# roclark/torchsr

Hardware: AMD Instinct MI355X
Metric: 96x96 HR crops/sec (SRGAN GAN train step) (higher is better)
Workload: dtype f32; 1 GPU; SRGAN full GAN step (Generator + Discriminator + VGG19 perceptual loss), 96x96 HR crops, batch 16 per GPU, fp32; per_gpu_batch=16, global_batch=16, crop=96, parallelism=dp1, hip_graph=True, vgg19_weights=seeded-random, plan_cus=256

## Files before the change

include/srx.h:

```cpp
#ifndef SRX_H
#define SRX_H

#include <stddef.h>
#include <stdint.h>

#ifdef __cplusplus
extern "C" {
#endif

#define SRX_VERSION 100

enum {
  SRX_OK = 0,
  SRX_E_BADARG = 1,
  SRX_E_UNSUPPORTED = 2,
  SRX_E_HIP = 3,
  SRX_E_WORKSPACE = 4
};

enum { SRX_ACT_NONE = 0, SRX_ACT_RELU = 1, SRX_ACT_LRELU = 2, SRX_ACT_PRELU = 3 };

int srx_version(void);
int srx_last_error(char* buf, size_t n);
int srx_build_info(char* buf, size_t n);
// ... 228 lines not shown
int srx_linear_bwd_data(const float* dy, const float* w, float* dx, int B, int K, int J, float* ws,
                        size_t ws_floats, void* stream);
int srx_linear_bwd_weight(const float* x, const float* dy, float* dw, int accumulate, int B, int K, int J,
                          void* stream);

int srx_mse_fwd(const float* a, const float* b, float* loss, int64_t n, float* ws, void* stream);
int srx_l1_fwd(const float* a, const float* b, float* loss, int64_t n, float* ws, void* stream);
int srx_mse_bwd(const float* a, const float* b, const float* gscale, float* da, float* db, int64_t n, void* stream);
int srx_l1_bwd(const float* a, const float* b, const float* gscale, float* da, float* db, int64_t n, void* stream);
int srx_l1_fwd_count(const float* a, const float* b, float* loss, int64_t n, int64_t count, float* ws, void* stream);
int srx_l1_bwd_count(const float* a, const float* b, const float* gscale, float* da, float* db, int64_t n, int64_t count,
                     void* stream);
int srx_bce_fwd(const float* p, float target, float* loss, int64_t n, float* ws, void* stream);
int srx_bce_bwd(const float* p, float target, const float* gscale, float* dp, int64_t n, void* stream);
int srx_bce_logits_fwd(const float* x, const float* shift, float target, float* loss, int64_t n, float* ws, void* stream);
int srx_bce_logits_bwd(const float* x, const float* shift, float target, const float* gscale, float* dx, int64_t n, void* stream);
int srx_mean_fwd(const float* x, float* out, int64_t n, float* ws, void* stream);
int srx_mean_bwd(const float* x, const float* gscale, float* dx, int64_t n, void* stream);

enum { SRX_HEAD_SRGAN_D = 0, SRX_HEAD_SRGAN_G = 1, SRX_HEAD_ESRGAN_D = 2, SRX_HEAD_ESRGAN_G = 3 };
typedef struct {
  int32_t mode, B, J, n_first;
  float slope, adv_weight;
} srx_gan_head_t;
int srx_gan_head_fwd(const srx_gan_head_t* h, const float* hidden, const float* w2, const float* b2, const float* shift,
                     const float* addend, float* zp, float* out, float* loss, void* stream);
int srx_gan_head_bwd(const srx_gan_head_t* h, const float* hidden, const float* w2, const float* zp, const float* out,
                     const float* shift, const float* g, float* dpre, float* dw2, float* db2, float* db1, int accumulate,
                     void* stream);

int srx_adam_step(float* p, const float* g, float* m, float* v, int64_t n, const float* lr, float beta1,
                  float beta2, float eps, float grad_scale, int64_t* step, void* stream);

#ifdef __cplusplus
}
#endif
#endif
```

torchsr_amd/_lib.py:

```python
import ctypes as C
import os
import subprocess
import sys

_HERE = os.path.dirname(os.path.abspath(__file__))
CSRC = os.path.join(_HERE, 'csrc')
LIB_PATH = os.environ.get('SRX_LIB') or os.path.join(CSRC, 'libsrx_hip.so')
SOURCES = ['api.cpp', 'gconv.hip', 'wgrad.hip', 'convpack.hip', 'c64.hip', 'thin9.hip', 'rdb.hip', 'thin.hip', 'rowtile.hip', 'augment.hip', 'norm.hip', 'eltwise.hip', 'linear.hip', 'loss.hip', 'head.hip', 'wino.hip', 'optim.hip']
HEADERS = ['srx_common.h', 'conv_host.h', os.path.join('..', '..', 'include', 'srx.h')]

ACT_NONE, ACT_RELU, ACT_LRELU, ACT_PRELU = 0, 1, 2, 3


class Conv2dDesc(C.Structure):
    _fields_ = [
        ('N', C.c_int32), ('H', C.c_int32), ('W', C.c_int32),
        ('Cin', C.c_int32), ('Cin_s', C.c_int32), ('Cout', C.c_int32), ('Cout_s', C.c_int32),
        ('KH', C.c_int32), ('KW', C.c_int32), ('stride', C.c_int32), ('pad', C.c_int32),
        ('shuffle', C.c_int32), ('act', C.c_int32), ('slope', C.c_float), ('up', C.c_int32),
        ('precision', C.c_int32),
    ]


class DgradEpilogue(C.Structure):
# ... 210 lines not shown
    'srx_mse_bwd': (_I, [_P, _P, _P, _P, _P, _L, _P]),
    'srx_l1_bwd': (_I, [_P, _P, _P, _P, _P, _L, _P]),
    'srx_l1_fwd_count': (_I, [_P, _P, _P, _L, _L, _P, _P]),
    'srx_l1_bwd_count': (_I, [_P, _P, _P, _P, _P, _L, _L, _P]),
    'srx_bce_fwd': (_I, [_P, _F, _P, _L, _P, _P]),
    'srx_bce_bwd': (_I, [_P, _F, _P, _P, _L, _P]),
    'srx_bce_logits_fwd': (_I, [_P, _P, _F, _P, _L, _P, _P]),
    'srx_bce_logits_bwd': (_I, [_P, _P, _F, _P, _P, _L, _P]),
    'srx_wino_applicable': (_I, [_D]),
    'srx_wino_packed_floats': (_Z, [_D]),
    'srx_wino_ws_floats': (_Z, [_D, _I]),
    'srx_wino_plan': (_I, [_D, _I, C.POINTER(C.c_int)]),
    'srx_wino_pack': (_I, [_D, _P, _P, _I, _P]),
    'srx_wino_fwd': (_I, [_D, _P, _P, _P, _P, _P, _Z, _P]),
    'srx_wino_bwd_data': (_I, [_D, _P, _P, _P, _P, _P, _Z, _P]),
    'srx_conv3x3_bf16s_applicable': (_I, [_D]),
    'srx_conv3x3_bf16s_packed_bytes': (_Z, [_D]),
    'srx_conv3x3_bf16s_pack': (_I, [_D, _P, _P, _P, _P]),
    'srx_conv3x3_bf16s_ws_floats': (_Z, [_D, _I]),
    'srx_conv3x3_bf16s_fwd': (_I, [_D, _P, _P, _P, _I, _P, _I, _P, _Z, _P]),
    'srx_conv3x3_bf16s_bwd_data': (_I, [_D, _P, _P, _P, _P, _I, _P, _Z, _P]),
    'srx_conv2d_fwd_first3_to_bf16': (_I, [_D, _P, _P, _P, _P, _P]),
    'srx_maxpool2x2_fwd_to_bf16': (_I, [_P, _P, _I, _I, _I, _I, _P]),
    'srx_maxpool2x2_relu_bwd_bf16': (_I, [_P, _P, _P, _I, _I, _I, _I, _P]),
    'srx_act_bwd_from_out_to_bf16': (_I, [_P, _P, _P, C.c_int64, _I, C.c_float, _P]),
    'srx_wino_infer_applicable': (_I, [_D]),
    'srx_wino_fwd_act': (_I, [_D, _P, _P, _P, _P, _P, _P, _Z, _P]),
    'srx_wino_force_plan': (_I, [_I, _I, _I]),
    'srx_wino_stat_rows': (_I, [_D]),
    'srx_wino_fwd_stats': (_I, [_D, _P, _P, _P, _P, _P, _P, _Z, _P]),
    'srx_gan_head_fwd': (_I, [C.POINTER(GanHead), _P, _P, _P, _P, _P, _P, _P, _P, _P]),
    'srx_gan_head_bwd': (_I, [C.POINTER(GanHead), _P, _P, _P, _P, _P, _P, _P, _P, _P, _P, _I, _P]),
    'srx_adam_step': (_I, [_P, _P, _P, _P, _L, _P, _F, _F, _F, _F, _P, _P]),
}
_UNCHECKED = {'srx_wino_applicable', 'srx_wino_infer_applicable', 'srx_conv3x3_bf16s_applicable', 'srx_wino_stat_rows', 'srx_conv2d_bwd_data_bn_rows', 'srx_conv2d_fwd_bn_in_ok', 'srx_conv2d_bwd_data_bn_in_ok', 'srx_pack_table_bytes', 'srx_version', 'srx_last_error', 'srx_device_cus', 'srx_plan_cus', 'srx_prof_stop', 'srx_conv2d_stat_rows', 'srx_bn_stat_rows', 'srx_bn_rows_per_block'}

EXPORTS = tuple(_SIGS.keys())

_lib = None


def load_handle(path: str) -> C.CDLL:
    import torch
    if torch.cuda.is_available():
        torch.cuda.init()
    return C.CDLL(path)


def _ensure_fresh():
    want = source_digest()
    if built_digest(LIB_PATH) == want:
        return
    import fcntl
    with open(os.path.join(CSRC, '.build.lock'), 'w') as lock:
        fcntl.flock(lock, fcntl.LOCK_EX)
        if built_digest(LIB_PATH) == want:
            return
        have = built_digest(LIB_PATH)
        print(f'torchsr_amd: {LIB_PATH} was built from other sources ({have and have[:12]} != {want[:12]}); rebuilding',
              file=sys.stderr)
        try:
            build()
        except (OSError, subprocess.CalledProcessError) as exc:
            raise RuntimeError(f'{LIB_PATH} is stale (built from sources {have and have[:12]}, the tree has {want[:12]}) and '
                               f'could not be rebuilt: {exc}.  Run `python -c "import __graft_entry__ as g; g.build()"`.') from exc


def lib() -> C.CDLL:
# ... 35 lines not shown
```

torchsr_amd/csrc/convpack.hip:

```cpp
#include "conv_host.h"

namespace {

__global__ void pack_fwd_kernel(const float* __restrict__ w, float* __restrict__ p, int Cout, int Cin, int KH, int KW,
                                int Ck, int K, int Kp, int Cnp, int shuffle_cps) {
  const int64_t idx = (int64_t)blockIdx.x * blockDim.x + threadIdx.x;
  if (idx >= (int64_t)Cnp * Kp) return;
  const int np = (int)(idx / Kp), k = (int)(idx - (int64_t)np * Kp);
  float v = 0.f;
  if (np < Cout && k < K) {
    const int tap = k / Ck, ci = k - tap * Ck;
    if (ci < Cin) {
      int co = np;
      if (shuffle_cps) { const int ij = np / shuffle_cps, cc = np - ij * shuffle_cps; co = cc * 4 + ij; }
      const int kh = tap / KW, kw = tap - kh * KW;
      v = w[(((size_t)co * Cin + ci) * KH + kh) * KW + kw];
    }
  }
  p[idx] = v;
}

__global__ void pack_bwd_kernel(const float* __restrict__ w, float* __restrict__ p, int Cout, int Cin, int KH, int KW,
                                int stride, int pad, int ph, int pw, int dminh, int dminw, int ntw, int Ck, int K,
                                int Kp, int Cnp, int shuffle_cps) {
// ... 196 lines not shown
      r.rows = Cnp; r.K = cls[c].K; r.Kp = cls[c].Kp; r.Ck = bwd_ck(d);
      r.ph = cls[c].ph; r.pw = cls[c].pw; r.dminh = cls[c].dminh; r.dminw = cls[c].dminw;
      r.ntw = cls[c].ntw > 0 ? cls[c].ntw : 1;
      r.n_elems = (long long)Cnp * (r.Ck + cls[c].Kp - cls[c].K);
      emit(r);
    }
  }
  *nrec_out = nrec;
  *max_elems_out = maxn;
  return SRX_OK;
}

extern "C" int srx_pack_table_add_wino(void* host_table, int* nrec, long long* max_elems, const srx_conv2d_t* d, const float* w,
                                       float* upk, int transpose) {
  SRX_REQUIRE(host_table && nrec && max_elems && d && w && upk && *nrec >= 0, "pack_table_add_wino: bad argument");
  SRX_REQUIRE(srx_wino_applicable(d) || srx_wino_packed_floats(d) > 0, "pack_table_add_wino: not a Winograd layer");
  PackRec r{};
  SRX_REQUIRE(!(transpose && d->shuffle), "pack_table_add_wino: a PixelShuffle layer has no Winograd data gradient");
  r.dst = upk; r.w = w; r.kind = transpose ? 5 : (d->shuffle ? 6 : 4);
  r.Cout = d->Cout; r.Cin = d->Cin; r.KH = 3; r.KW = 3; r.stride = 1; r.pad = 1;
  r.n_elems = (long long)d->Cout * d->Cin;
  static_cast<PackRec*>(host_table)[(*nrec)++] = r;
  if (r.n_elems > *max_elems) *max_elems = r.n_elems;
  return SRX_OK;
}

extern "C" int srx_pack_table_run(const void* dev_table, int nrec, long long max_elems, void* stream) {
  SRX_REQUIRE(dev_table && nrec > 0 && nrec <= 65535 && max_elems > 0, "pack_table_run: bad argument");
  hipLaunchKernelGGL(pack_table_kernel, dim3((unsigned)srx_cdiv(max_elems, 256), (unsigned)nrec), dim3(256), 0,
                     srx_stream(stream), static_cast<const PackRec*>(dev_table));
  SRX_CHECK_LAUNCH("pack_table_kernel");
  return SRX_OK;
}
```

torchsr_amd/csrc/optim.hip:

```cpp
#include "srx_common.h"

namespace {

__global__ void adam_tick_kernel(int64_t* step) { *step += 1; }

__global__ __launch_bounds__(256) void adam_kernel(float* __restrict__ p, const float* __restrict__ g,
                                                   float* __restrict__ m, float* __restrict__ v, int64_t n,
                                                   const float* __restrict__ lr_ptr, float beta1, float beta2,
                                                   float eps, float gscale, const int64_t* __restrict__ step_ptr) {
  const double t = (double)(*step_ptr);
  const float bc1 = (float)(1.0 - pow((double)beta1, t));
  const float bc2 = (float)(1.0 - pow((double)beta2, t));
  const float step_size = lr_ptr[0] / bc1;
  const float bc2_sqrt = sqrtf(bc2);
  const int64_t n4 = n / 4;
  for (int64_t i = (int64_t)blockIdx.x * blockDim.x + threadIdx.x; i < n4; i += (int64_t)gridDim.x * blockDim.x) {
    f32x4 pv = *reinterpret_cast<const f32x4*>(p + i * 4);
    f32x4 gv = *reinterpret_cast<const f32x4*>(g + i * 4);
    f32x4 mv = *reinterpret_cast<const f32x4*>(m + i * 4);
    f32x4 vv = *reinterpret_cast<const f32x4*>(v + i * 4);
#pragma unroll
    for (int e = 0; e < 4; ++e) {
      const float gg = gv[e] * gscale;
      mv[e] = beta1 * mv[e] + (1.f - beta1) * gg;
      vv[e] = beta2 * vv[e] + (1.f - beta2) * gg * gg;
      const float denom = sqrtf(vv[e]) / bc2_sqrt + eps;
      pv[e] -= step_size * (mv[e] / denom);
    }
    *reinterpret_cast<f32x4*>(p + i * 4) = pv;
    *reinterpret_cast<f32x4*>(m + i * 4) = mv;
    *reinterpret_cast<f32x4*>(v + i * 4) = vv;
  }
  if (blockIdx.x == 0 && threadIdx.x < (n & 3)) {
    const int64_t i = n4 * 4 + threadIdx.x;
    const float gg = g[i] * gscale;
    const float mm = beta1 * m[i] + (1.f - beta1) * gg;
    const float vv = beta2 * v[i] + (1.f - beta2) * gg * gg;
    m[i] = mm;
    v[i] = vv;
    p[i] -= step_size * (mm / (sqrtf(vv) / bc2_sqrt + eps));
  }
}

}

extern "C" int srx_adam_step(float* p, const float* g, float* m, float* v, int64_t n, const float* lr, float beta1,
                             float beta2, float eps, float grad_scale, int64_t* step, void* stream) {
  SRX_REQUIRE(p && g && m && v && lr && step && n > 0, "adam_step: bad argument");
  SRX_REQUIRE(((uintptr_t)p % 16 == 0) && ((uintptr_t)g % 16 == 0) && ((uintptr_t)m % 16 == 0) &&
                  ((uintptr_t)v % 16 == 0),
              "adam_step: buffers must be 16-byte aligned");
  hipStream_t st = srx_stream(stream);
  hipLaunchKernelGGL(adam_tick_kernel, dim3(1), dim3(1), 0, st, step);
  SRX_CHECK_LAUNCH("adam_tick_kernel");
  int64_t blocks = srx_cdiv(n / 4, 256);
  if (blocks > 4096) blocks = 4096;
  if (blocks < 1) blocks = 1;
  hipLaunchKernelGGL(adam_kernel, dim3((unsigned)blocks), dim3(256), 0, st, p, g, m, v, n, lr, beta1, beta2, eps,
                     grad_scale, step);
  SRX_CHECK_LAUNCH("adam_kernel");
  return SRX_OK;
}
```

torchsr_amd/csrc/srx_common.h:

```cpp
#pragma once
#include <hip/hip_runtime.h>
#include <hip/hip_ext.h>
#include <stdint.h>
#include <stddef.h>
#include "../../include/srx.h"

typedef float f32x4 __attribute__((ext_vector_type(4)));
typedef float f32x16 __attribute__((ext_vector_type(16)));

void srx_set_error(const char* fmt, ...);

#define SRX_FAIL(code, ...)      \
  do {                           \
    srx_set_error(__VA_ARGS__);  \
    return (code);               \
  } while (0)

#define SRX_REQUIRE(cond, ...) \
  do {                         \
    if (!(cond)) SRX_FAIL(SRX_E_BADARG, __VA_ARGS__); \
  } while (0)

#define SRX_CHECK_LAUNCH(name)                                                        \
  do {                                                                                \
// ... 41 lines not shown
                        const float* res;
                        float* z_out; };
struct srx_rt36_bnb_t { const float* y; const float* mean; const float* invstd; const float* gamma; const float* beta;
                        const float* prelu; const float* sums; float inv_m; float* dy_out; };
int srx_rt36_run(const srx_conv2d_t* d, const float* in, const float* wpk, const float* bias, const float* residual,
                 float* out, float* part, int act, float slope, hipStream_t st, const srx_rt36_bn_t* bn = nullptr,
                 const srx_rt36_bnl_t* bnl = nullptr, const srx_rt36_bnb_t* bnb = nullptr);

static inline hipStream_t srx_stream(void* s) { return (hipStream_t)s; }
static inline int64_t srx_cdiv(int64_t a, int64_t b) { return (a + b - 1) / b; }
static inline int64_t srx_roundup(int64_t a, int64_t b) { return srx_cdiv(a, b) * b; }

__device__ __forceinline__ void srx_divmod(int m, int d, float inv_d, int& q, int& r) {
  q = __float2int_rz(__int2float_rn(m) * inv_d);
  r = m - q * d;
  if (r < 0) { q -= 1; r += d; }
  if (r >= d) { q += 1; r -= d; }
}

__device__ __forceinline__ __amdgpu_buffer_rsrc_t srx_rsrc(const void* p, unsigned bytes) {
  return __builtin_amdgcn_make_buffer_rsrc(const_cast<void*>(p), (short)0, (int)bytes, 0x00020000);
}
__device__ __forceinline__ f32x4 srx_bload(__amdgpu_buffer_rsrc_t r, unsigned voff, unsigned soff) {
  return __builtin_bit_cast(f32x4, __builtin_amdgcn_raw_buffer_load_b128(r, (int)voff, (int)soff, 0));
}
__device__ __forceinline__ int srx_uniform(int v) { return __builtin_amdgcn_readfirstlane(v); }

__device__ __forceinline__ float srx_wave_sum(float v) {
#pragma unroll
  for (int o = 32; o > 0; o >>= 1) v += __shfl_xor(v, o, 64);
  return v;
}

__device__ __forceinline__ void srx_wino_pack_one(const float* __restrict__ w, float* __restrict__ upk, int Cout, int Cin,
                                                  int transpose, int64_t idx) {
  const int R = transpose == 1 ? Cin : Cout, K = transpose == 1 ? Cout : Cin;
  const int r = (int)(idx / K), k = (int)(idx - (int64_t)r * K);
  const int rsrc = transpose == 2 ? (r % (Cout / 4)) * 4 + r / (Cout / 4) : r;
  float g[3][3];
#pragma unroll
  for (int i = 0; i < 3; ++i)
#pragma unroll
    for (int j = 0; j < 3; ++j)
      g[i][j] = transpose == 1 ? w[(((size_t)k * Cin + r) * 3 + (2 - i)) * 3 + (2 - j)] : w[(((size_t)rsrc * Cin + k) * 3 + i) * 3 + j];
  float t[4][3];
#pragma unroll
  for (int j = 0; j < 3; ++j) {
    t[0][j] = g[0][j];
    t[1][j] = 0.5f * (g[0][j] + g[1][j] + g[2][j]);
    t[2][j] = 0.5f * (g[0][j] - g[1][j] + g[2][j]);
    t[3][j] = g[2][j];
  }
  const int nch = K / 32, rt = R / 32;
  const int jg = r >> 5, mrow = r & 31, kc = k / 32, kk = k % 32, quad = kk >> 2, e = kk & 3, s = quad >> 1, hh = quad & 1;
#pragma unroll
  for (int i = 0; i < 4; ++i) {
    const float u[4] = {t[i][0], 0.5f * (t[i][0] + t[i][1] + t[i][2]), 0.5f * (t[i][0] - t[i][1] + t[i][2]), t[i][2]};
#pragma unroll
    for (int j = 0; j < 4; ++j) {
      const int xi = 4 * i + j;
      upk[(((((size_t)xi * rt + jg) * nch + kc) * 4 + s) * 64 + hh * 32 + mrow) * 4 + e] = u[j];
    }
  }
}
```

torchsr_amd/functional.py:

```python
import contextlib
from typing import Optional, Tuple

import torch
from torch import Tensor
from torch.autograd import Function

from . import _dev, _lib
from ._lib import (ACT_LRELU, ACT_NONE, ACT_PRELU, ACT_RELU, HEAD_ESRGAN_D, HEAD_ESRGAN_G, HEAD_SRGAN_D, HEAD_SRGAN_G,
                   Conv2dDesc, call)

import ctypes as C


direct_grads = [False]


def _sink(param: Optional[Tensor]) -> Optional[Tensor]:
    if not direct_grads[0] or param is None or not param.requires_grad:
        return None
    g = param.grad
    if g is None or not g.is_cuda or g.dtype != torch.float32 or not g.is_contiguous():
        return None
    return g

# ... 319 lines not shown

    def pack_bf16s(self, weight: Tensor, d: Conv2dDesc, need_bwd: bool) -> None:
        key = self.pack_key(weight)
        have = self.__dict__.get('bf16s_fwd')
        if key == self.__dict__.get('_bf16s_key') and have is not None and (self.__dict__.get('bf16s_bwd') is not None or not need_bwd):
            return
        dref = C.byref(d)
        n = _lib.lib().srx_conv3x3_bf16s_packed_bytes(dref) // 2
        if have is None or have.device != weight.device:
            self.bf16s_fwd = torch.empty(n, dtype=torch.bfloat16, device=weight.device)
            self.bf16s_bwd = None
        if need_bwd and self.__dict__.get('bf16s_bwd') is None:
            self.bf16s_bwd = torch.empty(n, dtype=torch.bfloat16, device=weight.device)
        w = _chk(weight.detach(), 'conv2d.weight')
        call('srx_conv3x3_bf16s_pack', dref, _p(w), _p(self.bf16s_fwd), _p(self.bf16s_bwd), _stream())
        self._bf16s_key = key


def wino_forward_only_ok(st: ConvState, d: Conv2dDesc) -> bool:
    return (not _dev.NO_WINO and st.shuffle == 2 and st.act == ACT_NONE and st.precision == 0
            and _lib.lib().srx_wino_infer_applicable(C.byref(d)) == 1)


def wino_layer_ok(st: ConvState, d: Conv2dDesc) -> bool:
    return (not _dev.NO_WINO and st.act in (ACT_NONE, ACT_RELU) and _lib.lib().srx_wino_applicable(C.byref(d)) == 1)


def wino_forward_runs(st: ConvState, d: Conv2dDesc, want_stats: bool) -> bool:
    return wino_layer_ok(st, d) and (not want_stats or st.act == ACT_NONE)


class PackTable:

    def __init__(self, convs):
        self.convs = list(convs)
        self.table = None
        self.nrec, self.maxn = 0, 0
        self.fused_sig = None
        self.generation = 0

    def _build(self) -> bool:
        every = [(c._st, c.weight) for c in self.convs if c.weight.requires_grad and not c._st.fused_only]
        direct = [(st, wt) for st, wt in every if st.wpk_fwd is not None and getattr(st, 'last_desc', None) is not None]
        wino = [(st, wt) for st, wt in every if st.__dict__.get('wino_fwd') is not None]
        seen = {id(st) for st, _ in direct} | {id(st) for st, _ in wino}
        if not direct or any(id(st) not in seen for st, _ in every):
            return False
        items = direct
        n = len(items)
        descs = (Conv2dDesc * n)(*[st.last_desc for st, _ in items])
        arr = lambda ptrs: (C.c_void_p * n)(*ptrs)
        w, f, b = (arr([wt.data_ptr() for _, wt in items]), arr([st.wpk_fwd.data_ptr() for st, _ in items]),
                   arr([st.wpk_bwd.data_ptr() for st, _ in items]))
        nbytes = _lib.lib().srx_pack_table_bytes(n + len(wino))
        host = torch.empty(nbytes, dtype=torch.uint8)
        nrec, maxn = C.c_int(0), C.c_longlong(0)
        call('srx_pack_table_build', descs, n, w, f, b, host.data_ptr(), C.byref(nrec), C.byref(maxn))
        self.wino_items = wino
        for st, wt in self.wino_items:
            dref = C.byref(st._wino_desc)
            call('srx_pack_table_add_wino', host.data_ptr(), C.byref(nrec), C.byref(maxn), dref, wt.data_ptr(), st.wino_fwd.data_ptr(), 0)
            if st.wino_bwd is not None:
                call('srx_pack_table_add_wino', host.data_ptr(), C.byref(nrec), C.byref(maxn), dref, wt.data_ptr(), st.wino_bwd.data_ptr(), 1)
        self.table = host.to(items[0][1].device)
        self.items, self.nrec, self.maxn = items, nrec.value, maxn.value
        self.fused_sig = self._fused_signature()
        self.generation += 1
        return True

    def _fused_signature(self):
        return tuple((bool(c._st.fused_only), c._st.wpk_fwd is not None, c._st.__dict__.get('wino_fwd') is not None,
                      c._st.__dict__.get('wino_bwd') is not None) for c in self.convs)

    def run(self) -> bool:
        if self.table is not None and self.fused_sig != self._fused_signature():
            if torch.cuda.is_current_stream_capturing():
                raise RuntimeError('PackTable: the set of fused-only convs changed inside a hipGraph capture; run one eager step '
                                   'after switching precision / SRX_NO_RDB_FUSED')
            self.table = None
        if self.table is None and (torch.cuda.is_current_stream_capturing() or not self._build()):
            return False
        call('srx_pack_table_run', self.table.data_ptr(), self.nrec, self.maxn, _stream())
        for st, wt in self.items:
            st._key = st.pack_key(wt)
        for st, wt in self.wino_items:
            st._wino_key = st.pack_key(wt)
        return True


_pack_epoch = [0]


def bump_pack_epoch() -> None:
    _pack_epoch[0] += 1


class ActFold:
    __slots__ = ('act', 'slope', 'masked', 'consumers')

    def __init__(self, act: int, slope: float):
        self.act, self.slope, self.masked, self.consumers = act, float(slope), False, 0


class _Conv2d(Function):
    @staticmethod
    def forward(ctx, x: Tensor, weight: Tensor, bias: Optional[Tensor], st: ConvState, want_stats: bool,
                master: Tensor, in_act: Optional[ActFold] = None, act_bwd_folded: Optional[ActFold] = None):
        ctx.set_materialize_grads(False)
        if in_act is not None:
            if not isinstance(in_act, ActFold):
                raise TypeError('conv2d: in_act must be the ActFold token the producer was called with')
            in_act.consumers += 1
            if in_act.consumers > 1:
                raise RuntimeError('conv2d: an ActFold token has one consumer; this producer output feeds a second conv')
        if act_bwd_folded is not None and not isinstance(act_bwd_folded, ActFold):
            raise TypeError('conv2d: act_bwd_folded must be an ActFold token shared with the consumer')
        ctx.in_act, ctx.act_bwd_folded = in_act, act_bwd_folded
        x = _chk(x, 'conv2d.input')
        n, h, w, cs = x.shape
# ... 1645 lines not shown
```

torchsr_amd/optim.py:

```python
from typing import Iterable, List

import torch
from torch import nn, Tensor

from . import functional as F
from ._lib import call


class FlatParams:

    ALIGN = 4

    def __init__(self, module: nn.Module):
        params = [p for p in module.parameters() if p.requires_grad]
        if not params:
            raise RuntimeError('FlatParams: module has no trainable parameters')
        dev, dt = params[0].device, params[0].dtype
        if dt != torch.float32:
            raise RuntimeError('FlatParams: fp32 parameters expected')
        offs, total = [], 0
        for p in params:
            offs.append(total)
            total += (p.numel() + self.ALIGN - 1) // self.ALIGN * self.ALIGN
        self.data = torch.zeros(total, dtype=dt, device=dev)
# ... 10 lines not shown
            for p, o in zip(params, offs):
                n = p.numel()
                self.data[o:o + n].copy_(p.detach().reshape(-1))
                p.data = self.data[o:o + n].view(p.shape)
                p.grad = self.grad[o:o + n].view(p.shape)

    def offsets_by_name(self, module: nn.Module) -> dict:
        where = {id(p): o for p, o in zip(self.params, self.offsets)}
        return {n: where[id(p)] for n, p in module.named_parameters() if id(p) in where}

    def zero_grad(self) -> None:
        self.grad.zero_()
        off = 0
        for p in self.params:
            n = p.numel()
            if p.grad is None or p.grad.data_ptr() != self.grad.data_ptr() + off * 4:
                p.grad = self.grad[off:off + n].view(p.shape)
            off += (n + self.ALIGN - 1) // self.ALIGN * self.ALIGN


class FlatAdam:

    def __init__(self, flat: FlatParams, lr: float = 1e-4, betas=(0.9, 0.999), eps: float = 1e-8):
        self.flat = flat
        self.betas, self.eps = betas, eps
        dev = flat.data.device
        self.exp_avg = torch.zeros_like(flat.data)
        self.exp_avg_sq = torch.zeros_like(flat.data)
        self.step_count = torch.zeros((), dtype=torch.int64, device=dev)
        self.lr_dev = torch.tensor(float(lr), dtype=torch.float32, device=dev)
        self._lr = float(lr)
        self.grad_scale = 1.0
        self.pack_table = None
        self.param_groups = [{'lr': float(lr), 'initial_lr': float(lr)}]

    @property
    def lr(self) -> float:
        return self._lr

    def set_lr(self, lr: float) -> None:
        self._lr = float(lr)
        self.param_groups[0]['lr'] = float(lr)
        self.lr_dev.fill_(float(lr))

    def zero_grad(self) -> None:
        self.flat.zero_grad()

    @torch.no_grad()
    def step(self) -> None:
        f = self.flat
        call('srx_adam_step', f.data.data_ptr(), f.grad.data_ptr(), self.exp_avg.data_ptr(),
             self.exp_avg_sq.data_ptr(), f.numel, self.lr_dev.data_ptr(), self.betas[0], self.betas[1], self.eps,
             self.grad_scale, self.step_count.data_ptr(), torch.cuda.current_stream().cuda_stream)
        self.flat.pack_epoch[0] += 1
        if self.pack_table is not None:
            self.pack_table.run()

    def state_dict(self):
        return {'exp_avg': self.exp_avg, 'exp_avg_sq': self.exp_avg_sq, 'step': self.step_count, 'lr': self._lr}

    def load_state_dict(self, sd) -> None:
        self.exp_avg.copy_(sd['exp_avg'])
        self.exp_avg_sq.copy_(sd['exp_avg_sq'])
        self.step_count.copy_(sd['step'])
        self.set_lr(sd['lr'])


class StepLR:

    def __init__(self, optimizer: FlatAdam, step_size: int, gamma: float = 0.1):
        self.optimizer, self.step_size, self.gamma = optimizer, max(1, int(step_size)), gamma
        self.base_lr = optimizer.lr
        self.last_epoch = 0

    def step(self) -> None:
        self.last_epoch += 1
        self.optimizer.set_lr(self.base_lr * self.gamma ** (self.last_epoch // self.step_size))

    def get_last_lr(self):
        return [self.optimizer.lr]

    def state_dict(self):
        return {'last_epoch': self.last_epoch, 'base_lr': self.base_lr}

    def load_state_dict(self, sd) -> None:
        self.last_epoch, self.base_lr = sd['last_epoch'], sd['base_lr']
# ... 2 lines not shown
```

torchsr_amd/srgan/trainer.py:

```python
import os
import time
from argparse import Namespace
from math import log10
from typing import Callable, Dict, Optional

import torch
import torch.distributed as dist
from torch import Tensor

from .. import _dev
from .. import functional as F
from ..ddp import BackwardCuts, GradBuckets, broadcast_module
from ..layers import no_weight_grad, set_conv_precision
from ..optim import FlatAdam, FlatParams, StepLR
from .discriminator import Discriminator
from .generator import Generator
from .loss import VGGLoss

try:
    import wandb
except ImportError:
    wandb = None


# ... 126 lines not shown
        precision = 'bf16' if (self.amp and phase in self.amp_phases) else 'fp32'
        for module in (self.generator, self.discriminator, self.vgg_loss):
            set_conv_precision(module, precision)

    def _initialize_models(self) -> None:
        self.generator = self.generator_cls().to(self.device)
        self.discriminator = self.discriminator_cls().to(self.device)
        if self.distributed:
            broadcast_module(self.generator)
            broadcast_module(self.discriminator)
        self.gen_flat = FlatParams(self.generator)
        self.disc_flat = FlatParams(self.discriminator)
        force = self.force_collectives
        kw = {'force': force, 'reserve_cus': self.comm_reserved_cus, 'window_hook': self.comm_window_hook}
        self.gen_sync = GradBuckets(self.gen_flat, (self.gen_tail_bucket,), self.generator, **kw) if self.distributed else None
        self.disc_sync = GradBuckets(self.disc_flat, (self.disc_head_bucket,), self.discriminator, **kw) \
            if self.distributed else None

    def _initialize_loss(self) -> None:
        self.mse_loss = F.mse_loss
        self.pixel_loss = F.mse_loss
        self.bce_loss = F.bce_loss
        self.vgg_loss = VGGLoss(weights=self.vgg_weights).to(self.device)

    def _initialize_optimizers(self) -> None:
        self.psnr_optimizer = FlatAdam(self.gen_flat, lr=0.0001, betas=(0.9, 0.999))
        self.disc_optimizer = FlatAdam(self.disc_flat, lr=0.0001, betas=(0.9, 0.999))
        self.gen_optimizer = FlatAdam(self.gen_flat, lr=0.0001, betas=(0.9, 0.999))
        if self.distributed:
            for opt in (self.psnr_optimizer, self.gen_optimizer):
                opt.grad_scale = self.gen_sync.scale
            self.disc_optimizer.grad_scale = self.disc_sync.scale
        from ..layers import Conv2d
        gen_table = F.PackTable(m for m in self.generator.modules() if isinstance(m, Conv2d))
        disc_table = F.PackTable(m for m in self.discriminator.modules() if isinstance(m, Conv2d))
        self.psnr_optimizer.pack_table = self.gen_optimizer.pack_table = gen_table
        self.disc_optimizer.pack_table = disc_table
        self.disc_scheduler = StepLR(self.disc_optimizer, step_size=self.epochs // 8, gamma=0.6)
        self.gen_scheduler = StepLR(self.gen_optimizer, step_size=self.epochs // 8, gamma=0.6)

    def _create_test_image(self) -> None:
        path = 'media/waterfalls-low-res.png'
        if os.path.exists(path):
            import numpy as np
            from PIL import Image
            a = np.asarray(Image.open(path).convert('RGB'), dtype='float32') / 255.0
            image = torch.from_numpy(a).permute(2, 0, 1).contiguous()
        else:
            yy, xx = torch.meshgrid(torch.linspace(0, 1, 320), torch.linspace(0, 1, 480), indexing='ij')
            image = torch.stack([xx, yy, 0.5 + 0.5 * torch.sin(12 * xx * yy)])
        self.test_image = image.unsqueeze(0).to(self.device)

    def _log(self, statement: str) -> None:
        if self.main_process:
            print(statement)

    def _log_wandb(self, contents: dict, step: int = None) -> None:
        if wandb and self.main_process and getattr(wandb, 'run', None) is not None:
            wandb.log({k: (v.item() if torch.is_tensor(v) else v) for k, v in contents.items()}, step=step)

    def _cleanup(self) -> None:
        if wandb and getattr(wandb, 'run', None) is not None:
            wandb.finish()

    def _model_state(self, epoch: int, phase: str) -> dict:
        cpu = lambda sd: {k: (v.detach().clone().cpu() if torch.is_tensor(v) else v) for k, v in sd.items()}
        return {'epoch': epoch, 'phase': phase, 'state': cpu(self.generator.state_dict()),
                'resume': {'discriminator': cpu(self.discriminator.state_dict()),
# ... 391 lines not shown
```

Measured before the change: 2431 crops/s.

## Fuse Adam update with conv weight repacking into one table-driven kernel

Adds a table-driven kernel that runs the Adam update over the flat parameter buffer and, for conv layers, stages the updated weights in LDS and scatters them straight into the forward, data-gradient and Winograd packed layouts. This replaces the separate Adam pass plus pack-table pass, so the weights are not read from global memory a second time and one launch is saved. In exchange it needs a complex per-workgroup work table built on the host and heavier tail work per conv workgroup, with scattered stores into the packed layouts.

New measurement: 2441 crops/s, median of 6. About the same (+0.4%).

```diff
diff --git a/include/srx.h b/include/srx.h
--- a/include/srx.h
+++ b/include/srx.h
@@ -284,6 +284,13 @@
 int srx_adam_step(float* p, const float* g, float* m, float* v, int64_t n, const float* lr, float beta1,
                   float beta2, float eps, float grad_scale, int64_t* step, void* stream);
 
+size_t srx_pack_table_adam_bytes(const srx_conv2d_t* descs, int n_layers, long long total);
+int srx_pack_table_adam_build(const srx_conv2d_t* descs, int n_layers, const long long* w_off, long long total,
+                              float* const* wpk_fwd, float* const* wpk_bwd, float* const* wino_fwd, float* const* wino_bwd,
+                              void* host_table, size_t table_bytes, int* n_workgroups);
+int srx_pack_table_adam(float* p, const float* g, float* m, float* v, int64_t n, const float* lr, float beta1, float beta2,
+                        float eps, float grad_scale, int64_t* step, const void* dev_table, int n_workgroups, void* stream);
+
 #ifdef __cplusplus
 }
 #endif
diff --git a/torchsr_amd/_lib.py b/torchsr_amd/_lib.py
--- a/torchsr_amd/_lib.py
+++ b/torchsr_amd/_lib.py
@@ -266,8 +266,11 @@
     'srx_gan_head_fwd': (_I, [C.POINTER(GanHead), _P, _P, _P, _P, _P, _P, _P, _P, _P]),
     'srx_gan_head_bwd': (_I, [C.POINTER(GanHead), _P, _P, _P, _P, _P, _P, _P, _P, _P, _P, _I, _P]),
     'srx_adam_step': (_I, [_P, _P, _P, _P, _L, _P, _F, _F, _F, _F, _P, _P]),
+    'srx_pack_table_adam_bytes': (_Z, [_P, _I, C.c_longlong]),
+    'srx_pack_table_adam_build': (_I, [_P, _I, _P, C.c_longlong, _P, _P, _P, _P, _P, _Z, C.POINTER(C.c_int)]),
+    'srx_pack_table_adam': (_I, [_P, _P, _P, _P, _L, _P, _F, _F, _F, _F, _P, _P, _I, _P]),
 }
-_UNCHECKED = {'srx_wino_applicable', 'srx_wino_infer_applicable', 'srx_conv3x3_bf16s_applicable', 'srx_wino_stat_rows', 'srx_conv2d_bwd_data_bn_rows', 'srx_conv2d_fwd_bn_in_ok', 'srx_conv2d_bwd_data_bn_in_ok', 'srx_pack_table_bytes', 'srx_version', 'srx_last_error', 'srx_device_cus', 'srx_plan_cus', 'srx_prof_stop', 'srx_conv2d_stat_rows', 'srx_bn_stat_rows', 'srx_bn_rows_per_block'}
+_UNCHECKED = {'srx_wino_applicable', 'srx_wino_infer_applicable', 'srx_conv3x3_bf16s_applicable', 'srx_wino_stat_rows', 'srx_conv2d_bwd_data_bn_rows', 'srx_conv2d_fwd_bn_in_ok', 'srx_conv2d_bwd_data_bn_in_ok', 'srx_pack_table_bytes', 'srx_pack_table_adam_bytes', 'srx_version', 'srx_last_error', 'srx_device_cus', 'srx_plan_cus', 'srx_prof_stop', 'srx_conv2d_stat_rows', 'srx_bn_stat_rows', 'srx_bn_rows_per_block'}
 
 EXPORTS = tuple(_SIGS.keys())
 
diff --git a/torchsr_amd/csrc/convpack.hip b/torchsr_amd/csrc/convpack.hip
--- a/torchsr_amd/csrc/convpack.hip
+++ b/torchsr_amd/csrc/convpack.hip
@@ -252,3 +252,130 @@
   SRX_CHECK_LAUNCH("pack_table_kernel");
   return SRX_OK;
 }
+
+namespace {
+int adam_pack_per_wg(int taps) { return taps * 256 <= SRX_AP_LDS ? 256 : (SRX_AP_LDS / taps) & ~3; }
+long long adam_pack_conv_wgs(const srx_conv2d_t* d) {
+  return srx_cdiv((long long)d->Cout * d->Cin, adam_pack_per_wg(d->KH * d->KW));
+}
+}
+
+extern "C" size_t srx_pack_table_adam_bytes(const srx_conv2d_t* descs, int n, long long total) {
+  if (!descs || n <= 0 || total <= 0) return 0;
+  long long nwork = 0, ntap = 0;
+  for (int i = 0; i < n; ++i) {
+    if (descs[i].KH <= 0 || descs[i].KW <= 0 || descs[i].KH * descs[i].KW > SRX_AP_LDS / 4) return 0;
+    nwork += adam_pack_conv_wgs(descs + i);
+    ntap += descs[i].KH * descs[i].KW;
+  }
+  nwork += srx_cdiv(total, SRX_AP_PLAIN) + n + 1;
+  return sizeof(SrxAdamPackHead) + (size_t)nwork * sizeof(SrxAdamPackWork) + (size_t)n * sizeof(SrxAdamPackLayer) +
+         (size_t)ntap * sizeof(SrxAdamPackTap);
+}
+
+extern "C" int srx_pack_table_adam_build(const srx_conv2d_t* descs, int n, const long long* w_off, long long total,
+                                         float* const* wpk_fwd, float* const* wpk_bwd, float* const* wino_fwd,
+                                         float* const* wino_bwd, void* host_table, size_t table_bytes, int* nwork_out) {
+  SRX_REQUIRE(descs && w_off && wpk_fwd && wpk_bwd && wino_fwd && wino_bwd && host_table && nwork_out && n > 0 && n < 32768,
+              "pack_table_adam_build: bad argument");
+  SRX_REQUIRE(total > 0 && total % 4 == 0, "pack_table_adam_build: the flat buffer must be a multiple of 4 floats");
+  SRX_REQUIRE(table_bytes >= srx_pack_table_adam_bytes(descs, n, total) && srx_pack_table_adam_bytes(descs, n, total) > 0,
+              "pack_table_adam_build: table buffer too small");
+  long long nwork = 0;
+  int ntap = 0;
+  long long at = 0;
+  for (int i = 0; i < n; ++i) {
+    const srx_conv2d_t* d = descs + i;
+    if (int rc = check_desc(d)) return rc;
+    const long long numel = (long long)d->Cout * d->Cin * d->KH * d->KW;
+    SRX_REQUIRE(w_off[i] % 4 == 0 && w_off[i] >= at && w_off[i] + numel <= total,
+                "pack_table_adam_build: layer %d lies outside the flat buffer, unaligned or out of order", i);
+    SRX_REQUIRE((long long)d->Cout * d->Cin < (1LL << 31), "pack_table_adam_build: layer %d too large", i);
+    nwork += srx_cdiv(w_off[i] - at, SRX_AP_PLAIN) + adam_pack_conv_wgs(d);
+    at = srx_roundup(w_off[i] + numel, 4);
+    SRX_REQUIRE(at <= total, "pack_table_adam_build: layer %d ends past the flat buffer", i);
+    ntap += d->KH * d->KW;
+  }
+  nwork += srx_cdiv(total - at, SRX_AP_PLAIN);
+  SRX_REQUIRE(nwork > 0 && nwork < (1LL << 31), "pack_table_adam_build: too many workgroups");
+  SrxAdamPackHead* hd = static_cast<SrxAdamPackHead*>(host_table);
+  *hd = SrxAdamPackHead{(int)nwork, n, ntap, 0, total, 0};
+  SrxAdamPackWork* work = reinterpret_cast<SrxAdamPackWork*>(hd + 1);
+  SrxAdamPackLayer* layers = reinterpret_cast<SrxAdamPackLayer*>(work + nwork);
+  SrxAdamPackTap* taps = reinterpret_cast<SrxAdamPackTap*>(layers + n);
+  long long iw = 0;
+  int it = 0;
+  auto plain = [&](long long from, long long to) {
+    for (long long b = from; b < to; b += SRX_AP_PLAIN) {
+      const long long len = to - b < SRX_AP_PLAIN ? to - b : (long long)SRX_AP_PLAIN;
+      work[iw++] = SrxAdamPackWork{b, (int)len, 0, (short)-1, (short)0};
+    }
+  };
+  at = 0;
+  for (int i = 0; i < n; ++i) {
+    const srx_conv2d_t* d = descs + i;
+    const int ntaps = d->KH * d->KW;
+    SrxAdamPackLayer L{};
+    L.Cout = d->Cout; L.Cin = d->Cin; L.taps = ntaps;
+    L.fwd_kind = L.bwd_kind = -1;
+    L.tap0 = it;
+    const Geo g = fwd_geo(d);
+    L.cps = g.cps;
+    if (wpk_fwd[i]) {
+      L.fwd = wpk_fwd[i];
+      if (srx_thin_fwd_applicable(d)) {
+        L.fwd_kind = 2;
+      } else {
+        L.fwd_kind = 0; L.fwd_Kp = g.Kp; L.fwd_Ck = g.Ck;
+      }
+    }
+    if (wpk_fwd[i] && wpk_bwd[i]) {
+      L.bwd = wpk_bwd[i];
+      if (srx_thin_dgrad_applicable(d)) {
+        L.bwd_kind = 3;
+      } else {
+        SRX_REQUIRE(d->stride <= 4, "pack_table_adam_build: stride > 4 unsupported for the data gradient");
+        L.bwd_kind = 1; L.bwd_Ck = bwd_ck(d);
+        BwdClass cls[16];
+        size_t tot;
+        const int nc = bwd_classes(d, cls, tot);
+        for (int t = 0; t < ntaps; ++t) taps[it + t] = SrxAdamPackTap{-1, 0};
+        for (int c = 0; c < nc; ++c)
+          for (int th = 0; th < cls[c].nth; ++th)
+            for (int tw = 0; tw < cls[c].ntw; ++tw) {
+              const int kh = cls[c].ph + d->pad - d->stride * (cls[c].dminh + th);
+              const int kw = cls[c].pw + d->pad - d->stride * (cls[c].dminw + tw);
+              SRX_REQUIRE(kh >= 0 && kh < d->KH && kw >= 0 && kw < d->KW && taps[it + kh * d->KW + kw].base < 0,
+                          "pack_table_adam_build: layer %d: a data-gradient class tap outside the filter or met twice", i);
+              const size_t base = cls[c].woff + (size_t)(th * cls[c].ntw + tw) * L.bwd_Ck;
+              SRX_REQUIRE(base + (size_t)pad_rows(d->Cin) * cls[c].Kp < (1ULL << 31), "pack_table_adam_build: layer %d: pack too large", i);
+              taps[it + kh * d->KW + kw] = SrxAdamPackTap{(int)base, cls[c].Kp};
+            }
+        for (int t = 0; t < ntaps; ++t)
+          SRX_REQUIRE(taps[it + t].base >= 0, "pack_table_adam_build: layer %d: tap %d belongs to no data-gradient class", i, t);
+      }
+    }
+    if (wino_fwd[i] || wino_bwd[i]) {
+      SRX_REQUIRE(srx_wino_packed_floats(d) > 0 && wino_fwd[i], "pack_table_adam_build: layer %d is not a Winograd layer", i);
+      SRX_REQUIRE(!(wino_bwd[i] && d->shuffle), "pack_table_adam_build: a PixelShuffle layer has no Winograd data gradient");
+      L.wino_f = wino_fwd[i]; L.wino_b = wino_bwd[i];
+    }
+    SRX_REQUIRE(L.fwd || L.wino_f, "pack_table_adam_build: layer %d has no packed copy", i);
+    it += ntaps;
+    layers[i] = L;
+    plain(at, w_off[i]);
+    const int per = adam_pack_per_wg(ntaps);
+    const long long filters = (long long)d->Cout * d->Cin, end4 = srx_roundup(w_off[i] + filters * ntaps, 4);
+    for (long long f = 0; f < filters; f += per) {
+      const int cnt = (int)(filters - f < per ? filters - f : per);
+      const long long b = w_off[i] + f * ntaps;
+      const long long len = f + cnt == filters ? end4 - b : (long long)cnt * ntaps;
+      work[iw++] = SrxAdamPackWork{b, (int)len, (int)f, (short)i, (short)cnt};
+    }
+    at = end4;
+  }
+  plain(at, total);
+  SRX_REQUIRE(iw == nwork && it == ntap, "pack_table_adam_build: internal count mismatch");
+  *nwork_out = (int)nwork;
+  return SRX_OK;
+}
diff --git a/torchsr_amd/csrc/optim.hip b/torchsr_amd/csrc/optim.hip
--- a/torchsr_amd/csrc/optim.hip
+++ b/torchsr_amd/csrc/optim.hip
@@ -4,15 +4,27 @@
 
 __global__ void adam_tick_kernel(int64_t* step) { *step += 1; }
 
+struct AdamCoef { float beta1, beta2, eps, gscale, step_size, bc2_sqrt; };
+__device__ __forceinline__ AdamCoef adam_coef(const float* __restrict__ lr_ptr, float beta1, float beta2, float eps, float gscale,
+                                              const int64_t* __restrict__ step_ptr) {
+  const double t = (double)(*step_ptr);
+  const float bc1 = (float)(1.0 - pow((double)beta1, t));
+  const float bc2 = (float)(1.0 - pow((double)beta2, t));
+  return AdamCoef{beta1, beta2, eps, gscale, lr_ptr[0] / bc1, sqrtf(bc2)};
+}
+__device__ __forceinline__ void adam_elem(float& p, float& m, float& v, float g, const AdamCoef& c) {
+  const float gg = g * c.gscale;
+  m = c.beta1 * m + (1.f - c.beta1) * gg;
+  v = c.beta2 * v + (1.f - c.beta2) * gg * gg;
+  const float denom = sqrtf(v) / c.bc2_sqrt + c.eps;
+  p -= c.step_size * (m / denom);
+}
+
 __global__ __launch_bounds__(256) void adam_kernel(float* __restrict__ p, const float* __restrict__ g,
                                                    float* __restrict__ m, float* __restrict__ v, int64_t n,
                                                    const float* __restrict__ lr_ptr, float beta1, float beta2,
                                                    float eps, float gscale, const int64_t* __restrict__ step_ptr) {
-  const double t = (double)(*step_ptr);
-  const float bc1 = (float)(1.0 - pow((double)beta1, t));
-  const float bc2 = (float)(1.0 - pow((double)beta2, t));
-  const float step_size = lr_ptr[0] / bc1;
-  const float bc2_sqrt = sqrtf(bc2);
+  const AdamCoef c = adam_coef(lr_ptr, beta1, beta2, eps, gscale, step_ptr);
   const int64_t n4 = n / 4;
   for (int64_t i = (int64_t)blockIdx.x * blockDim.x + threadIdx.x; i < n4; i += (int64_t)gridDim.x * blockDim.x) {
     f32x4 pv = *reinterpret_cast<const f32x4*>(p + i * 4);
@@ -21,11 +33,9 @@
     f32x4 vv = *reinterpret_cast<const f32x4*>(v + i * 4);
 #pragma unroll
     for (int e = 0; e < 4; ++e) {
-      const float gg = gv[e] * gscale;
-      mv[e] = beta1 * mv[e] + (1.f - beta1) * gg;
-      vv[e] = beta2 * vv[e] + (1.f - beta2) * gg * gg;
-      const float denom = sqrtf(vv[e]) / bc2_sqrt + eps;
-      pv[e] -= step_size * (mv[e] / denom);
+      float pe = pv[e], me = mv[e], ve = vv[e];
+      adam_elem(pe, me, ve, gv[e], c);
+      pv[e] = pe; mv[e] = me; vv[e] = ve;
     }
     *reinterpret_cast<f32x4*>(p + i * 4) = pv;
     *reinterpret_cast<f32x4*>(m + i * 4) = mv;
@@ -33,12 +43,74 @@
   }
   if (blockIdx.x == 0 && threadIdx.x < (n & 3)) {
     const int64_t i = n4 * 4 + threadIdx.x;
-    const float gg = g[i] * gscale;
-    const float mm = beta1 * m[i] + (1.f - beta1) * gg;
-    const float vv = beta2 * v[i] + (1.f - beta2) * gg * gg;
+    float pp = p[i], mm = m[i], vv = v[i];
+    adam_elem(pp, mm, vv, g[i], c);
     m[i] = mm;
     v[i] = vv;
-    p[i] -= step_size * (mm / (sqrtf(vv) / bc2_sqrt + eps));
+    p[i] = pp;
+  }
+}
+
+__global__ __launch_bounds__(256) void adam_pack_kernel(float* __restrict__ p, const float* __restrict__ g, float* __restrict__ m,
+                                                        float* __restrict__ v, const float* __restrict__ lr_ptr, float beta1,
+                                                        float beta2, float eps, float gscale,
+                                                        const int64_t* __restrict__ step_ptr, const char* __restrict__ blob) {
+  __shared__ __attribute__((aligned(16))) float sw[SRX_AP_LDS + 4];
+  const SrxAdamPackHead* hd = reinterpret_cast<const SrxAdamPackHead*>(blob);
+  const SrxAdamPackWork* works = reinterpret_cast<const SrxAdamPackWork*>(hd + 1);
+  const SrxAdamPackWork wk = works[blockIdx.x];
+  const AdamCoef c = adam_coef(lr_ptr, beta1, beta2, eps, gscale, step_ptr);
+  const bool conv = wk.layer >= 0;
+  const int n4 = wk.n / 4;
+  for (int i = threadIdx.x; i < n4; i += 256) {
+    const int64_t at = wk.base + (int64_t)i * 4;
+    f32x4 pv = *reinterpret_cast<const f32x4*>(p + at);
+    f32x4 gv = *reinterpret_cast<const f32x4*>(g + at);
+    f32x4 mv = *reinterpret_cast<const f32x4*>(m + at);
+    f32x4 vv = *reinterpret_cast<const f32x4*>(v + at);
+#pragma unroll
+    for (int e = 0; e < 4; ++e) {
+      float pe = pv[e], me = mv[e], ve = vv[e];
+      adam_elem(pe, me, ve, gv[e], c);
+      pv[e] = pe; mv[e] = me; vv[e] = ve;
+    }
+    *reinterpret_cast<f32x4*>(p + at) = pv;
+    *reinterpret_cast<f32x4*>(m + at) = mv;
+    *reinterpret_cast<f32x4*>(v + at) = vv;
+    if (conv) *reinterpret_cast<f32x4*>(sw + i * 4) = pv;
+  }
+  if (!conv) return;
+  __syncthreads();
+  if ((int)threadIdx.x >= wk.count) return;
+  const SrxAdamPackLayer* layers = reinterpret_cast<const SrxAdamPackLayer*>(works + hd->nwork);
+  const SrxAdamPackTap* tp = reinterpret_cast<const SrxAdamPackTap*>(layers + hd->nlayer);
+  const SrxAdamPackLayer L = layers[wk.layer];
+  const int f = wk.first + threadIdx.x;
+  const int co = f / L.Cin, ci = f - co * L.Cin;
+  const float* mine = sw + threadIdx.x * L.taps;
+  for (int t0 = 0; t0 < L.taps; t0 += 9) {
+    float w9[9];
+#pragma unroll
+    for (int u = 0; u < 9; ++u) w9[u] = mine[min(t0 + u, L.taps - 1)];
+    if (L.fwd_kind >= 0) {
+#pragma unroll
+      for (int u = 0; u < 9; ++u)
+        if (t0 + u < L.taps) L.fwd[srx_ap_fwd_index(L, co, ci, t0 + u)] = w9[u];
+    }
+    if (L.bwd_kind >= 0) {
+#pragma unroll
+      for (int u = 0; u < 9; ++u)
+        if (t0 + u < L.taps) L.bwd[srx_ap_bwd_index(L, tp, co, ci, t0 + u)] = w9[u];
+    }
+    if (L.taps == 9) {
+      if (L.wino_f) srx_wino_scatter(w9, L.wino_f, L.Cout, L.Cin, srx_ap_row(co, L.cps), ci);
+      if (L.wino_b) {
+        float r9[9];
+#pragma unroll
+        for (int u = 0; u < 9; ++u) r9[u] = w9[8 - u];
+        srx_wino_scatter(r9, L.wino_b, L.Cin, L.Cout, ci, co);
+      }
+    }
   }
 }
 
@@ -61,3 +133,19 @@
   SRX_CHECK_LAUNCH("adam_kernel");
   return SRX_OK;
 }
+
+extern "C" int srx_pack_table_adam(float* p, const float* g, float* m, float* v, int64_t n, const float* lr, float beta1,
+                                   float beta2, float eps, float grad_scale, int64_t* step, const void* table, int nwork,
+                                   void* stream) {
+  SRX_REQUIRE(p && g && m && v && lr && step && table && n > 0 && n % 4 == 0 && nwork > 0, "pack_table_adam: bad argument");
+  SRX_REQUIRE(((uintptr_t)p % 16 == 0) && ((uintptr_t)g % 16 == 0) && ((uintptr_t)m % 16 == 0) &&
+                  ((uintptr_t)v % 16 == 0) && ((uintptr_t)table % 16 == 0),
+              "pack_table_adam: buffers must be 16-byte aligned");
+  hipStream_t st = srx_stream(stream);
+  hipLaunchKernelGGL(adam_tick_kernel, dim3(1), dim3(1), 0, st, step);
+  SRX_CHECK_LAUNCH("adam_tick_kernel");
+  hipLaunchKernelGGL(adam_pack_kernel, dim3((unsigned)nwork), dim3(256), 0, st, p, g, m, v, lr, beta1, beta2, eps, grad_scale,
+                     step, static_cast<const char*>(table));
+  SRX_CHECK_LAUNCH("adam_pack_kernel");
+  return SRX_OK;
+}
diff --git a/torchsr_amd/csrc/srx_common.h b/torchsr_amd/csrc/srx_common.h
--- a/torchsr_amd/csrc/srx_common.h
+++ b/torchsr_amd/csrc/srx_common.h
@@ -97,34 +97,72 @@
   return v;
 }
 
+__host__ __device__ __forceinline__ size_t srx_wino_index(int xi, int R, int K, int r, int k) {
+  const int nch = K / 32, rt = R / 32;
+  const int jg = r >> 5, mrow = r & 31, kc = k / 32, kk = k % 32, quad = kk >> 2, e = kk & 3, s = quad >> 1, hh = quad & 1;
+  return (((((size_t)xi * rt + jg) * nch + kc) * 4 + s) * 64 + hh * 32 + mrow) * 4 + e;
+}
+__device__ __forceinline__ void srx_wino_scatter(const float* g, float* __restrict__ upk, int R, int K, int r, int k) {
+  float t[4][3];
+#pragma unroll
+  for (int j = 0; j < 3; ++j) {
+    t[0][j] = g[j];
+    t[1][j] = 0.5f * (g[j] + g[3 + j] + g[6 + j]);
+    t[2][j] = 0.5f * (g[j] - g[3 + j] + g[6 + j]);
+    t[3][j] = g[6 + j];
+  }
+#pragma unroll
+  for (int i = 0; i < 4; ++i) {
+    const float u[4] = {t[i][0], 0.5f * (t[i][0] + t[i][1] + t[i][2]), 0.5f * (t[i][0] - t[i][1] + t[i][2]), t[i][2]};
+#pragma unroll
+    for (int j = 0; j < 4; ++j) upk[srx_wino_index(4 * i + j, R, K, r, k)] = u[j];
+  }
+}
+
 __device__ __forceinline__ void srx_wino_pack_one(const float* __restrict__ w, float* __restrict__ upk, int Cout, int Cin,
                                                   int transpose, int64_t idx) {
   const int R = transpose == 1 ? Cin : Cout, K = transpose == 1 ? Cout : Cin;
   const int r = (int)(idx / K), k = (int)(idx - (int64_t)r * K);
   const int rsrc = transpose == 2 ? (r % (Cout / 4)) * 4 + r / (Cout / 4) : r;
-  float g[3][3];
+  float g[9];
 #pragma unroll
   for (int i = 0; i < 3; ++i)
 #pragma unroll
     for (int j = 0; j < 3; ++j)
-      g[i][j] = transpose == 1 ? w[(((size_t)k * Cin + r) * 3 + (2 - i)) * 3 + (2 - j)] : w[(((size_t)rsrc * Cin + k) * 3 + i) * 3 + j];
-  float t[4][3];
-#pragma unroll
-  for (int j = 0; j < 3; ++j) {
-    t[0][j] = g[0][j];
-    t[1][j] = 0.5f * (g[0][j] + g[1][j] + g[2][j]);
-    t[2][j] = 0.5f * (g[0][j] - g[1][j] + g[2][j]);
-    t[3][j] = g[2][j];
-  }
-  const int nch = K / 32, rt = R / 32;
-  const int jg = r >> 5, mrow = r & 31, kc = k / 32, kk = k % 32, quad = kk >> 2, e = kk & 3, s = quad >> 1, hh = quad & 1;
-#pragma unroll
-  for (int i = 0; i < 4; ++i) {
-    const float u[4] = {t[i][0], 0.5f * (t[i][0] + t[i][1] + t[i][2]), 0.5f * (t[i][0] - t[i][1] + t[i][2]), t[i][2]};
-#pragma unroll
-    for (int j = 0; j < 4; ++j) {
-      const int xi = 4 * i + j;
-      upk[(((((size_t)xi * rt + jg) * nch + kc) * 4 + s) * 64 + hh * 32 + mrow) * 4 + e] = u[j];
-    }
-  }
+      g[3 * i + j] = transpose == 1 ? w[(((size_t)k * Cin + r) * 3 + (2 - i)) * 3 + (2 - j)] : w[(((size_t)rsrc * Cin + k) * 3 + i) * 3 + j];
+  srx_wino_scatter(g, upk, R, K, r, k);
 }
+
+constexpr int SRX_AP_LDS = 2592;
+constexpr int SRX_AP_PLAIN = 4096;
+struct SrxAdamPackHead { int nwork, nlayer, ntap, pad_; long long total, pad2_; };
+struct SrxAdamPackWork {
+  long long base;
+  int n;
+  int first;
+  short layer;
+  short count;
+};
+struct SrxAdamPackLayer {
+  float* fwd;
+  float* bwd;
+  float* wino_f;
+  float* wino_b;
+  int Cout, Cin, taps, cps;
+  int fwd_kind, fwd_Kp, fwd_Ck;
+  int bwd_kind, bwd_Ck;
+  int tap0;
+  int pad_;
+};
+struct SrxAdamPackTap { int base, Kp; };
+
+__host__ __device__ __forceinline__ int srx_ap_row(int co, int cps) { return cps ? (co & 3) * cps + (co >> 2) : co; }
+__host__ __device__ __forceinline__ size_t srx_ap_fwd_index(const SrxAdamPackLayer& L, int co, int ci, int tap) {
+  if (L.fwd_kind == 2) return ((size_t)co * L.taps + tap) * 64 + ci;
+  return (size_t)srx_ap_row(co, L.cps) * L.fwd_Kp + (size_t)tap * L.fwd_Ck + ci;
+}
+__host__ __device__ __forceinline__ size_t srx_ap_bwd_index(const SrxAdamPackLayer& L, const SrxAdamPackTap* tp, int co, int ci, int tap) {
+  if (L.bwd_kind == 3) return ((size_t)ci * L.taps + (L.taps - 1 - tap)) * 64 + co;
+  const SrxAdamPackTap t = tp[L.tap0 + tap];
+  return (size_t)t.base + (size_t)ci * t.Kp + srx_ap_row(co, L.cps);
+}
diff --git a/torchsr_amd/functional.py b/torchsr_amd/functional.py
--- a/torchsr_amd/functional.py
+++ b/torchsr_amd/functional.py
@@ -375,9 +375,11 @@
 
 class PackTable:
 
-    def __init__(self, convs):
+    def __init__(self, convs, flat=None):
         self.convs = list(convs)
+        self.flat = flat
         self.table = None
+        self.adam_table, self.adam_nwork = None, 0
         self.nrec, self.maxn = 0, 0
         self.fused_sig = None
         self.generation = 0
@@ -407,27 +409,63 @@
                 call('srx_pack_table_add_wino', host.data_ptr(), C.byref(nrec), C.byref(maxn), dref, wt.data_ptr(), st.wino_bwd.data_ptr(), 1)
         self.table = host.to(items[0][1].device)
         self.items, self.nrec, self.maxn = items, nrec.value, maxn.value
+        self.adam_table, self.adam_nwork = self._build_adam(every, {id(st) for st, _ in direct})
         self.fused_sig = self._fused_signature()
         self.generation += 1
         return True
 
+    def _build_adam(self, every, direct):
+        flat = self.flat
+        if flat is None:
+            return None, 0
+        where = {id(p): o for p, o in zip(flat.params, flat.offsets)}
+        base = flat.data.data_ptr()
+        rows = []
+        for st, wt in every:
+            off = where.get(id(wt))
+            if off is None or wt.data_ptr() != base + 4 * off or not wt.is_contiguous():
+                return None, 0
+            have_direct, have_wino = id(st) in direct, st.__dict__.get('wino_fwd') is not None
+            rows.append((off, st.last_desc if have_direct else st._wino_desc,
+                         st.wpk_fwd.data_ptr() if have_direct else None, st.wpk_bwd.data_ptr() if have_direct else None,
+                         st.wino_fwd.data_ptr() if have_wino else None,
+                         st.wino_bwd.data_ptr() if have_wino and st.wino_bwd is not None else None))
+        rows.sort(key=lambda r: r[0])
+        n = len(rows)
+        descs = (Conv2dDesc * n)(*[r[1] for r in rows])
+        offs = (C.c_longlong * n)(*[r[0] for r in rows])
+        ptrs = [(C.c_void_p * n)(*[r[k] for r in rows]) for k in (2, 3, 4, 5)]
+        nbytes = _lib.lib().srx_pack_table_adam_bytes(descs, n, flat.numel)
+        if nbytes == 0:
+            return None, 0
+        host = torch.zeros(nbytes, dtype=torch.uint8)
+        nwork = C.c_int(0)
+        call('srx_pack_table_adam_build', descs, n, offs, flat.numel, *ptrs, host.data_ptr(), nbytes, C.byref(nwork))
+        return host.to(flat.data.device), nwork.value
+
     def _fused_signature(self):
         return tuple((bool(c._st.fused_only), c._st.wpk_fwd is not None, c._st.__dict__.get('wino_fwd') is not None,
                       c._st.__dict__.get('wino_bwd') is not None) for c in self.convs)
 
-    def run(self) -> bool:
+    def ready(self) -> bool:
         if self.table is not None and self.fused_sig != self._fused_signature():
             if torch.cuda.is_current_stream_capturing():
                 raise RuntimeError('PackTable: the set of fused-only convs changed inside a hipGraph capture; run one eager step '
                                    'after switching precision / SRX_NO_RDB_FUSED')
-            self.table = None
-        if self.table is None and (torch.cuda.is_current_stream_capturing() or not self._build()):
-            return False
-        call('srx_pack_table_run', self.table.data_ptr(), self.nrec, self.maxn, _stream())
+            self.table = self.adam_table = None
+        return not (self.table is None and (torch.cuda.is_current_stream_capturing() or not self._build()))
+
+    def stamp(self) -> None:
         for st, wt in self.items:
             st._key = st.pack_key(wt)
         for st, wt in self.wino_items:
             st._wino_key = st.pack_key(wt)
+
+    def run(self) -> bool:
+        if not self.ready():
+            return False
+        call('srx_pack_table_run', self.table.data_ptr(), self.nrec, self.maxn, _stream())
+        self.stamp()
         return True
 
 
diff --git a/torchsr_amd/optim.py b/torchsr_amd/optim.py
--- a/torchsr_amd/optim.py
+++ b/torchsr_amd/optim.py
@@ -66,6 +66,7 @@
         self._lr = float(lr)
         self.grad_scale = 1.0
         self.pack_table = None
+        self.fuse_pack = True
         self.param_groups = [{'lr': float(lr), 'initial_lr': float(lr)}]
 
     @property
@@ -83,9 +84,19 @@
     @torch.no_grad()
     def step(self) -> None:
         f = self.flat
+        table = self.pack_table
+        stream = torch.cuda.current_stream().cuda_stream
+        if (self.fuse_pack and table is not None and table.flat is f and table.table is not None and table.ready()
+                and table.adam_table is not None):
+            call('srx_pack_table_adam', f.data.data_ptr(), f.grad.data_ptr(), self.exp_avg.data_ptr(),
+                 self.exp_avg_sq.data_ptr(), f.numel, self.lr_dev.data_ptr(), self.betas[0], self.betas[1], self.eps,
+                 self.grad_scale, self.step_count.data_ptr(), table.adam_table.data_ptr(), table.adam_nwork, stream)
+            f.pack_epoch[0] += 1
+            table.stamp()
+            return
         call('srx_adam_step', f.data.data_ptr(), f.grad.data_ptr(), self.exp_avg.data_ptr(),
              self.exp_avg_sq.data_ptr(), f.numel, self.lr_dev.data_ptr(), self.betas[0], self.betas[1], self.eps,
-             self.grad_scale, self.step_count.data_ptr(), torch.cuda.current_stream().cuda_stream)
+             self.grad_scale, self.step_count.data_ptr(), stream)
         self.flat.pack_epoch[0] += 1
         if self.pack_table is not None:
             self.pack_table.run()
diff --git a/torchsr_amd/srgan/trainer.py b/torchsr_amd/srgan/trainer.py
--- a/torchsr_amd/srgan/trainer.py
+++ b/torchsr_amd/srgan/trainer.py
@@ -182,8 +182,8 @@
                 opt.grad_scale = self.gen_sync.scale
             self.disc_optimizer.grad_scale = self.disc_sync.scale
         from ..layers import Conv2d
-        gen_table = F.PackTable(m for m in self.generator.modules() if isinstance(m, Conv2d))
-        disc_table = F.PackTable(m for m in self.discriminator.modules() if isinstance(m, Conv2d))
+        gen_table = F.PackTable((m for m in self.generator.modules() if isinstance(m, Conv2d)), flat=self.gen_flat)
+        disc_table = F.PackTable((m for m in self.discriminator.modules() if isinstance(m, Conv2d)), flat=self.disc_flat)
         self.psnr_optimizer.pack_table = self.gen_optimizer.pack_table = gen_table
         self.disc_optimizer.pack_table = disc_table
         self.disc_scheduler = StepLR(self.disc_optimizer, step_size=self.epochs // 8, gamma=0.6)
```
